# christopherkarani/Wax

Measured on NVIDIA H100. Metric: queries/sec cosine top-10 @ 10Mx384 fp32, higher is better.
Workload: dtype f32

## Files before the change

### wax_b200/csrc/waxvs_batch.cuh

```cuda
#pragma once
#include <cuda.h>
#include <cuda_bf16.h>

#include "waxvs_common.cuh"
#include "waxvs_scan.cuh"

namespace waxvs {

constexpr int kBatchM = 128;
constexpr int kBatchN = 128;
constexpr int kBatchKBlock = 32;
constexpr int kBatchKBlockBf16 = 64;
constexpr int kBatchRescore = 256;
constexpr int kBatchRescoreMax = 1024;
constexpr uint32_t kBatchABytes = kBatchM * 128u;
constexpr uint32_t kBatchBBytes = kBatchN * 128u;
constexpr uint32_t kBatchStageBytes = kBatchABytes + kBatchBBytes;
constexpr int kBatchStageSlots = 8;
constexpr uint32_t kBatchScoreStride = kBatchN + 8;
constexpr uint32_t kBatchScoreBytes = kBatchM * kBatchScoreStride * 4u;
constexpr int kBatchMaxStages = 6;
constexpr uint32_t kBatchSmemOptin = 227u * 1024u;
__host__ __device__ constexpr uint32_t batch_smem_bytes(int stages, int heap, uint32_t ares_kb = 0) {
    return ares_kb * kBatchABytes + stages * (ares_kb ? kBatchBBytes : kBatchStageBytes) + kBatchScoreBytes +
// ... 897 lines not shown
            const float scale = METRIC == kCosine ? qn : qn * __uint_as_float(*p.max_norm_bits);
            const float sk_exact = METRIC == kCosine ? (1.0f - dk) * qn : 1.0f - dk;
            const float acc_slack = static_cast<float>(p.dims) * 0x1p-23f * scale;
            const float ulp_slack = 0x1p-21f * fmaxf(1.0f, fabsf(dk)) * (METRIC == kCosine ? qn : 1.0f);
            const float eps = p.eps_rel * scale * 1.01f + acc_slack + ulp_slack + 1e-30f;
            if (excluded_any && (!(sk_exact > tau + eps) || !finite_f32(eps))) ok = 0;
            const float feps = kTf32Eps * scale * 1.01f + acc_slack + ulp_slack + 1e-30f;
            const float t = sk_exact - feps;
            tau_star = finite_f32(t) ? t - fabsf(t) * 0x1p-20f - 1e-30f : -INFINITY;
            const float feps16 = kBf16Eps * scale * 1.01f + acc_slack + ulp_slack + 1e-30f;
            const float t16 = sk_exact - feps16;
            tau_star16 = finite_f32(t16) ? t16 - fabsf(t16) * 0x1p-20f - 1e-30f : -INFINITY;
        } else if (excluded_any) {
            ok = 0;
        }
        if (METRIC != kL2 && (!(s_a2 >= 0x1p-126f) || !finite_f32(s_a2))) {
            ok = 0;
            tau_star = tau_star16 = -INFINITY;
        }
        p.ok[q] = ok;
        if (p.tau_star) { p.tau_star[q] = tau_star; p.tau_star[p.tau_stride + q] = tau_star16; }
    }
    ScanParams sp{};
    sp.out = p.out + static_cast<size_t>(q) * p.k;
    sp.frame_ids = p.frame_ids; sp.id_base = p.id_base; sp.row_offset = p.row_offset; sp.row_keys = p.row_keys;
    for (uint32_t i = threadIdx.x; i < p.k; i += blockDim.x)
        write_candidate(sp, static_cast<int>(i), i < p.rescore ? ek[i] : WAXVS_KEY_NONE);
}

struct RescoreParams {
    const float *corpus, *query;
    uint32_t dims, k, n_nominees;
    const uint64_t *nominees;
    uint32_t *aux;
    const uint32_t *max_norm_bits;
    float rho_max;
    uint64_t *block_keys;
    uint32_t *ticket;
    uint32_t *work_counter;
    wax_vs_candidate *out;
    uint32_t *ok;
    const uint64_t *frame_ids, *row_keys;
    uint64_t id_base, row_offset;
    uint32_t tail_smem_bytes;
};

template <int METRIC>
__global__ void __launch_bounds__(512, 1) shadow_rescore_kernel(const RescoreParams p) {
    static_assert(METRIC == kCosine || METRIC == kDot, "the shadow route covers cosine and dot");
    extern __shared__ __align__(16) unsigned char rsm[];
    __shared__ float s_a2, s_sqrt_a2;
    const int warp = threadIdx.x >> 5, lane = threadIdx.x & 31, warps = blockDim.x >> 5;
    const int k = static_cast<int>(p.k);
    if (warp == 0) {
        float s0 = 0.f, s1 = 0.f, s2 = 0.f, s3 = 0.f;
        for (uint32_t base = 4u * lane; base < p.dims; base += 128u) {
            const float4 x = __ldg(reinterpret_cast<const float4 *>(p.query + base));
            s0 = __fmaf_rn(x.x, x.x, s0); s1 = __fmaf_rn(x.y, x.y, s1);
            s2 = __fmaf_rn(x.z, x.z, s2); s3 = __fmaf_rn(x.w, x.w, s3);
        }
        const float a2 = warp_butterfly_sum(__fadd_rn(__fadd_rn(s0, s1), __fadd_rn(s2, s3)));
        if (lane == 0) { s_a2 = a2; s_sqrt_a2 = __fsqrt_rn(a2); }
    }
    __shared__ ScanParams sp;
    for (uint32_t i = threadIdx.x; i < sizeof(ScanParams) / 4u; i += blockDim.x) reinterpret_cast<uint32_t *>(&sp)[i] = 0u;
    __syncthreads();
    if (threadIdx.x == 0) {
        sp.k = p.k; sp.block_keys = p.block_keys; sp.ticket = p.ticket; sp.out = p.out;
        sp.frame_ids = p.frame_ids; sp.id_base = p.id_base; sp.row_offset = p.row_offset; sp.row_keys = p.row_keys;
        sp.tail_smem_bytes = p.tail_smem_bytes; sp.work_counter = p.work_counter;
    }
    __syncthreads();

    WarpTopK<1> tk;
    tk.init();
    const uint32_t stride = gridDim.x * warps * 4u;
    for (uint32_t i0 = (blockIdx.x * warps + warp) * 4u; i0 < p.n_nominees; i0 += stride) {
        uint64_t nk[4];
        const float *vp[4];
        float d[4];
#pragma unroll
        for (uint32_t r = 0; r < 4; ++r) {
            nk[r] = i0 + r < p.n_nominees ? p.nominees[i0 + r] : WAXVS_KEY_NONE;
            vp[r] = p.corpus + static_cast<size_t>(nk[r] == WAXVS_KEY_NONE ? 0u : static_cast<uint32_t>(nk[r])) * p.dims;
        }
        exact_row_distance_x4<METRIC>(p.query, vp, p.dims, s_a2, s_sqrt_a2, lane, d);
#pragma unroll
        for (uint32_t r = 0; r < 4; ++r) {
            if (nk[r] == WAXVS_KEY_NONE || !finite_f32(d[r])) continue;
            const uint64_t x = make_key(d[r], static_cast<uint32_t>(nk[r]));
            if (x < tk.thresh) tk.insert(x, lane, k);
        }
    }

    if (!finish_topk_select<1>(sp, tk, rsm)) return;
    __syncthreads();
    if (threadIdx.x != 0) return;
    const wax_vs_candidate kth = p.out[p.k - 1];
    const uint32_t cut = p.aux[0];
    const bool excluded_any = cut != WAXVS_UKEY_NONE;
    const float tau = excluded_any ? -from_orderable_u32(cut) : -INFINITY;
    const float rho_q = __uint_as_float(p.aux[1]);
    uint32_t ok = 1;
    if (kth.valid) {
        const float dk = kth.distance, qn = s_sqrt_a2;
        const float m = METRIC == kCosine ? 1.0f : __uint_as_float(*p.max_norm_bits);
        const float scale = qn * m;
        const float sk_exact = METRIC == kCosine ? (1.0f - dk) * qn : 1.0f - dk;
        const float coding = qn * p.rho_max + rho_q * ((METRIC == kCosine ? 1.0001f : m) + p.rho_max);
        const float acc_slack = static_cast<float>(p.dims) * 0x1p-23f * scale;
        const float ulp_slack = 0x1p-21f * fmaxf(1.0f, fabsf(dk)) * (METRIC == kCosine ? qn : 1.0f);
        const float eps = coding * 1.01f + acc_slack + ulp_slack + 1e-30f;
        if (excluded_any && (!(sk_exact > tau + eps) || !finite_f32(eps))) ok = 0;
    } else if (excluded_any) {
        ok = 0;
    }
    if (!(s_a2 >= 0x1p-126f) || !finite_f32(s_a2)) ok = 0;
    *p.ok = ok;
    p.aux[0] = WAXVS_UKEY_NONE;
    p.aux[2] = cut;
}

template <int METRIC>
__global__ void __launch_bounds__(256) filter_rescore_kernel(const float *corpus, const float *queries, uint32_t dims,
                                                             const uint32_t *cand_count, const uint32_t *cand_rows,
                                                             uint32_t cand_cap, uint64_t *keys) {
    const uint32_t q = blockIdx.y;
    const int lane = threadIdx.x & 31;
    const uint32_t n = min(cand_count[q], cand_cap);
    const uint32_t warps = (gridDim.x * blockDim.x) >> 5;
    uint32_t i = (blockIdx.x * blockDim.x + threadIdx.x) >> 5;
    if (i >= n) return;
    const float *qv = queries + static_cast<size_t>(q) * dims;
    float a2 = 0.0f, sqrt_a2 = 0.0f;
    if (METRIC == kCosine) {
        float s0 = 0.f, s1 = 0.f, s2 = 0.f, s3 = 0.f;
        for (uint32_t base = 4u * lane; base < dims; base += 128u) {
            const float x = __ldg(qv + base); s0 = __fmaf_rn(x, x, s0);
            if (base + 1 < dims) { const float y = __ldg(qv + base + 1); s1 = __fmaf_rn(y, y, s1); }
            if (base + 2 < dims) { const float z = __ldg(qv + base + 2); s2 = __fmaf_rn(z, z, s2); }
            if (base + 3 < dims) { const float w = __ldg(qv + base + 3); s3 = __fmaf_rn(w, w, s3); }
        }
        a2 = warp_butterfly_sum(__fadd_rn(__fadd_rn(s0, s1), __fadd_rn(s2, s3)));
        sqrt_a2 = __fsqrt_rn(a2);
    }
    for (uint32_t i0 = i; i0 < n; i0 += 4u * warps) {
        uint32_t rr[4];
        const float *vp[4];
        float d[4];
#pragma unroll
        for (uint32_t r = 0; r < 4; ++r) {
            const uint32_t j = i0 + r * warps;
            rr[r] = cand_rows[static_cast<size_t>(q) * cand_cap + (j < n ? j : i0)];
// ... 43 lines not shown
```

### wax_b200/csrc/waxvs_engine.cu

```cuda
#include <cuda_runtime.h>

#include <algorithm>
#include <atomic>
#include <cstdarg>
#include <cstdio>
#include <cstring>
#include <limits>
#include <map>
#include <mutex>
#include <new>
#include <shared_mutex>
#include <string>
#include <unordered_map>
#include <chrono>
#include <random>
#include <thread>
#include <unistd.h>
#include <cmath>
#include <vector>

#include "../../include/wax_vs_cuda.h"
#include "waxvs_common.cuh"
#include "waxvs_scan.cuh"
#include "waxvs_select.cuh"
// ... 780 lines not shown
}

constexpr uint32_t kShadowNominees = 128;
constexpr uint32_t kShadowRescore = 256;
constexpr uint32_t kShadowSkipQueries = 16;
static bool shadow_route_applies(const wax_vs_engine *e) {
    return e->tune.shadow_scan && (e->similarity == WAX_VS_COSINE || e->similarity == WAX_VS_DOT) && !e->debug_trace &&
           e->tune.batch_bf16 != 0 && e->dims % kBatchKBlockBf16 == 0 &&
           e->n_rows * e->dims * sizeof(float) >= e->tune.route[kRouteBf16].min_bytes;
}
static int32_t select_route_form(wax_vs_engine *e, cudaStream_t stream, bool demoted, bool *use, RouteForm *form,
                                 TmaConfig *cfg) {
    *use = false;
    for (const RouteForm f : {kRouteU4, kRouteInt8, kRouteBf16}) {
        if ((f == kRouteU4 && demoted) || e->n_rows * e->dims * sizeof(float) < e->tune.route[f].min_bytes ||
            !pick_route_config(e, f, cfg))
            continue;
        if (const int32_t rc = ensure_route_shadow(e, f, stream)) return rc;
        if (e->shadows[f].valid && e->shadows[f].eps_rel <= kRouteSpec[f].max_eps_rel) {
            *use = true;
            *form = f;
            return WAX_VS_OK;
        }
    }
    return WAX_VS_OK;
}

static int32_t enqueue_shadow_nominations(wax_vs_engine *e, SearchCtx *c, const ScanParams &p, const TmaConfig &cfg,
                                          cudaStream_t stream, uint64_t *launches, uint32_t *shape, RouteForm f) {
    const RouteFormSpec &fs = kRouteSpec[f];
    const wax_vs_engine::Shadow &sh = e->shadows[f];
    int32_t rc;
    if (fs.grid_rescore && !c->d_u4_aux) {
        if ((rc = c->d_u4_aux.ensure(3, "4-bit route state"))) return rc;
        CUDA_TRY(cudaMemsetAsync(c->d_u4_aux, 0xFF, 3 * sizeof(uint32_t), stream));
    }
    const size_t cta_keys = static_cast<size_t>(std::max(e->tune.grid, e->sm_count)) * kU4CtaNominees;
    if ((rc = c->d_heaps.ensure(std::max(static_cast<size_t>(kShadowNominees) * kNomineeStride, fs.grid_rescore ? cta_keys : 0), "nominee keys")) ||
        (rc = c->d_ok.ensure(1, "proof flags")) || (!p.query && (rc = c->d_queries.ensure(e->dims, "query buffer"))))
        return rc;

    ScanParams sp = p;
    sp.corpus = reinterpret_cast<const float *>(sh.codes.p);
    sp.row_scale = fs.scaled ? sh.scale.p : nullptr;
    sp.u4_aux = fs.grid_rescore ? c->d_u4_aux.p : nullptr;
    sp.k = kShadowNominees;
    sp.out = nullptr; sp.host_out = nullptr; sp.host_flag = nullptr;
    sp.nominees = c->d_heaps;
    sp.query_store = p.query ? nullptr : c->d_queries.p;
    sp.tail_select = e->tune.tail_select ? 1u : 0u;
    sp.tail_smem_bytes = static_cast<uint32_t>(static_cast<size_t>(cfg.warps) * cfg.stages * cfg.R * e->dims * fs.tail_bytes);
    const int grid = tma_grid(e, c, cfg, sp);
    CUDA_TRY(fs.launch(e, &sp, grid, cfg, e->similarity, stream));

    if (fs.grid_rescore) {
        RescoreParams rp{};
        rp.corpus = e->d_corpus; rp.query = p.query ? p.query : c->d_queries.p;
        rp.dims = e->dims; rp.k = p.k; rp.n_nominees = static_cast<uint32_t>(grid) * kU4CtaNominees;
        rp.nominees = c->d_heaps; rp.aux = c->d_u4_aux; rp.max_norm_bits = e->d_max_norm; rp.rho_max = sh.rho_max;
        rp.block_keys = c->d_block_keys; rp.ticket = c->d_ticket; rp.work_counter = sp.work_counter; rp.out = p.out; rp.ok = c->d_ok;
        rp.frame_ids = p.frame_ids; rp.id_base = p.id_base; rp.row_offset = p.row_offset; rp.row_keys = p.row_keys;
        rp.tail_smem_bytes = static_cast<uint32_t>(grid) * p.k * sizeof(uint64_t);
        if (rp.tail_smem_bytes > 48u * 1024u) rp.tail_smem_bytes = 0;
        const auto kernel = e->similarity == WAX_VS_COSINE ? shadow_rescore_kernel<kCosine> : shadow_rescore_kernel<kDot>;
        kernel<<<grid, 512, rp.tail_smem_bytes, stream>>>(rp);
        CUDA_TRY(cudaGetLastError());
    } else {
        FinishParams fp{};
        fp.corpus = e->d_corpus; fp.queries = p.query ? p.query : c->d_queries.p;
        fp.n_rows = p.n_rows; fp.dims = e->dims; fp.n_queries = 1; fp.groups = 1; fp.slices = 1;
        fp.kprime = kShadowNominees; fp.k = p.k; fp.metric = e->similarity;
        fp.heaps = c->d_heaps; fp.max_norm_bits = e->d_max_norm;
        fp.out = p.out; fp.ok = c->d_ok;
        fp.frame_ids = p.frame_ids; fp.id_base = p.id_base; fp.row_offset = p.row_offset; fp.row_keys = p.row_keys;
        fp.pow2_all = 512; fp.rescore = kShadowRescore; fp.eps_rel = sh.eps_rel;
        const size_t fsmem = static_cast<size_t>(fp.pow2_all + fp.rescore) * sizeof(uint64_t);
        const auto kernel = e->similarity == WAX_VS_COSINE ? batch_finish_kernel<kCosine> : batch_finish_kernel<kDot>;
        CUDA_TRY(grant_smem(e, kernel, fsmem));
        kernel<<<1, 512, fsmem, stream>>>(fp);
        CUDA_TRY(cudaGetLastError());
    }
    *launches += 2;
    if (shape) {
        const uint32_t s[7] = {static_cast<uint32_t>(cfg.C), static_cast<uint32_t>(cfg.R), static_cast<uint32_t>(cfg.warps),
                               static_cast<uint32_t>(cfg.stages), static_cast<uint32_t>(grid), sp.chunk_steps, sp.tail_select};
        std::copy(s, s + 7, shape);
    }
    return WAX_VS_OK;
}

static int32_t enqueue_shadow_route(wax_vs_engine *e, SearchCtx *c, ScanParams &p, cudaStream_t stream, uint64_t *launches) {
    if (!shadow_route_applies(e)) return WAX_VS_OK;
    int32_t rc;
    if (!c->h_proof_count) {
        if ((rc = c->d_proof_count.ensure(2, "proof counts")) || (rc = c->h_proof_count.ensure(2, "proof count mirror"))) return rc;
        CUDA_TRY(cudaMemsetAsync(c->d_proof_count, 0, 2 * sizeof(uint32_t), stream));
        c->h_proof_count[0] = c->h_proof_count[1] = 0;
        c->seen_failed = 0;
    }
    bool demoted;
    {
        std::lock_guard<std::mutex> pg(e->pool_mu);
        const uint32_t failed = *static_cast<volatile uint32_t *>(c->h_proof_count + 1);
        if (failed != c->seen_failed) {
            c->seen_failed = failed;
            if (c->last_u4) {
                if (e->u4_probing) e->u4_demote_window = std::min(e->u4_demote_window * 2, 1u << 20);
                e->u4_demoted = e->u4_demote_window;
            } else {
                e->shadow_scan_skip = kShadowSkipQueries;
            }
        } else if (c->last_u4 && e->u4_probing) {
            e->u4_demote_window = 16;
        }
        if (c->last_u4) e->u4_probing = false;
        c->last_u4 = false;
        if (e->shadow_scan_skip > 0) { --e->shadow_scan_skip; return WAX_VS_OK; }
        demoted = e->u4_demoted > 0;
        if (demoted && --e->u4_demoted == 0) e->u4_probing = true;
    }
    bool use = false;
    RouteForm form = kRouteBf16;
    TmaConfig cfg{};
    if ((rc = select_route_form(e, stream, demoted, &use, &form, &cfg)) || !use) return rc;
    if ((rc = enqueue_shadow_nominations(e, c, p, cfg, stream, launches, nullptr, form))) return rc;
    c->last_u4 = form == kRouteU4;
    {
        std::lock_guard<std::mutex> pg(e->pool_mu);
        ++e->single_route_queries[form];
    }
// ... 4630 lines not shown
    else if (!strcmp(name, "batch_bf16_queries")) *out = e->batch_bf16_queries;
    else if (!strcmp(name, "batch_retry_queries")) *out = e->batch_retry_queries;
    else if (!strcmp(name, "batch_filter_bf16_queries")) *out = e->batch_filter_bf16_queries;
    else if (!strcmp(name, "shadow_bytes")) *out = bf.valid ? bf.rows * e->dims * sizeof(__nv_bfloat16) : 0;
    else if (!strcmp(name, "shadow_capacity_bytes")) *out = bf.codes.cap * sizeof(uint32_t);
    else if (!strcmp(name, "shadow_unavailable")) *out = bf.unavailable ? 1 : 0;
    else if (!strcmp(name, "batch_tf32_queries")) *out = e->batch_tf32_queries;
    else if (!strcmp(name, "filter_bitset_passes")) *out = e->filter_bitset_passes;
    else if (!strcmp(name, "group_index_builds")) *out = e->group_index_builds;
    else if (!strcmp(name, "where_group_units")) *out = e->where_group_units;
    else if (!strcmp(name, "where_group_rows_walked")) *out = e->where_group_rows_walked;
    else if (!strcmp(name, "attribute_uploads")) *out = e->attribute_uploads;
    else if (!strcmp(name, "location_uploads")) *out = e->location_uploads;
    else if (!strcmp(name, "term_index_builds")) *out = e->term_index_builds;
    else if (!strcmp(name, "term_index_bytes"))
        *out = e->tindex.keys.cap * sizeof(uint64_t) + e->tindex.start.cap * sizeof(uint64_t) + e->tindex.postings.cap * sizeof(uint32_t);
    else if (!strcmp(name, "grouped_batch_covered_queries")) *out = e->grouped_batch_covered_queries;
    else if (!strcmp(name, "grouped_batch_expanded_groups")) *out = e->grouped_batch_expanded_groups;
    else if (!strcmp(name, "grouped_batch_fallback_queries")) *out = e->grouped_batch_fallback_queries;
    else if (!strcmp(name, "grouped_batch_expansion_passes")) *out = e->grouped_batch_expansion_passes;
    else if (!strcmp(name, "shard_grouped_expanded_groups")) *out = e->shard_grouped_expanded_groups;
    else if (!strcmp(name, "ingest_h2d_bytes")) *out = e->ingest_h2d_bytes;
    else if (!strcmp(name, "ingest_d2h_bytes")) *out = e->ingest_d2h_bytes;
    else if (!strcmp(name, "norms_rows")) *out = e->norms_rows;
    else if (!strcmp(name, "shadow_rows")) *out = bf.rows;
    else if (!strcmp(name, "int8_shadow_bytes")) *out = i8.valid ? i8.rows * (e->dims + sizeof(float)) : 0;
    else if (!strcmp(name, "int8_shadow_rows")) *out = i8.rows;
    else if (!strcmp(name, "u4_shadow_bytes")) *out = u4.valid ? u4.rows * (e->dims / 2 + sizeof(float)) : 0;
    else if (!strcmp(name, "u4_shadow_rows")) *out = u4.rows;
    else if (!strcmp(name, "single_u4_queries")) *out = e->single_route_queries[kRouteU4];
    else if (!strcmp(name, "single_int8_queries")) *out = e->single_route_queries[kRouteInt8];
    else if (!strcmp(name, "batch_heap_bump")) *out = e->heap_bump;
    else if (!strcmp(name, "batch_last_heap")) *out = e->last_heap;
    else if (!strcmp(name, "single_shadow_queries") || !strcmp(name, "single_shadow_fallbacks")) {
        const int slot = !strcmp(name, "single_shadow_queries") ? 0 : 1;
        uint64_t n = 0;
        auto add = [&](const SearchCtx *c) { if (c->h_proof_count) n += *static_cast<volatile uint32_t *>(c->h_proof_count + slot); };
        for (const SearchCtx *c : e->pool) add(c);
        for (const auto &kv : e->stream_ctx) add(kv.second);
        *out = n;
    }
    else if (!strcmp(name, "pool_allocs")) *out = e->pool_allocs;
    else if (!strcmp(name, "pool_reuses")) *out = e->pool_reuses;
    else return fail(WAX_VS_ERR_ARGUMENT, "unknown counter '%s'", name);
    return WAX_VS_OK;
}

int32_t wax_vs_debug_time_search_batch(wax_vs_engine *e, uint32_t n_queries, int64_t top_k, uint64_t seed,
                                       uint32_t warmup, uint32_t iters, float *out_ms_total,
                                       uint64_t *out_launches, uint32_t *out_unproven) {
    WAX_VS_MULTI_REFUSE(e, "wax_vs_debug_time_search_batch");
    if (!e || !out_ms_total) return fail(WAX_VS_ERR_NULL, "NULL argument");
    if (n_queries == 0) n_queries = 1;
    std::shared_lock<std::shared_mutex> r(e->rw);
    DeviceGuard g(e->device);
    const uint32_t k_eff = static_cast<uint32_t>(std::min<uint64_t>(clamp_topk(top_k), std::max<uint64_t>(e->n_rows, 1)));
    if (!batch_tensor_eligible(e, n_queries, k_eff))
        return fail(WAX_VS_ERR_UNSUPPORTED, "batch of %u queries, k=%u, dims=%u is not eligible for the tensor path", n_queries, k_eff, e->dims);
    CtxLease lease(e);
    int32_t rc = lease.acquire();
    if (rc) return rc;
    SearchCtx *c = lease.c;
    const size_t qfloats = static_cast<size_t>(n_queries) * e->dims;
    if ((rc = c->d_queries.ensure(qfloats, "query buffer"))) return rc;
    if ((rc = c->d_out.ensure(static_cast<size_t>(n_queries) * k_eff, "result buffer"))) return rc;
    if ((rc = c->d_ok.ensure(static_cast<size_t>(n_queries), "proof flags"))) return rc;
    if ((rc = c->h_ok.ensure(static_cast<size_t>(n_queries), "proof flag staging"))) return rc;
    synth_fill_kernel<<<(n_queries + 255) / 256, 256, 0, c->stream>>>(c->d_queries, n_queries, e->dims, seed, 0, 1);
// ... 86 lines not shown
        e->tune.batch_bf16 == 0 || e->dims % kBatchKBlockBf16 != 0 ||
        (form == kRouteBf16 && e->shadows[kRouteBf16].unavailable) || !pick_route_config(e, form, &cfg))
        return fail(WAX_VS_ERR_UNSUPPORTED, "no %s-shadow route for k=%u, dims=%u in this shape", fs.name, k_eff, e->dims);
    DeviceGuard g(e->device);
    if (!g.ok) return g.error();
    CtxLease lease(e);
    int32_t rc = lease.acquire();
    if (rc) return rc;
    SearchCtx *c = lease.c;
    if ((rc = ensure_route_shadow(e, form, c->stream, true))) return rc;
    if (!e->shadows[form].valid) return fail(WAX_VS_ERR_UNSUPPORTED, "the %s shadow does not fit in device memory", fs.name);
    if ((rc = c->d_out.ensure(k_eff, "result buffer"))) return rc;
    const uint32_t *d_mask = nullptr;
    if (allow_bits) {
        const size_t words = static_cast<size_t>((e->n_rows + 31) / 32);
        if ((rc = c->d_mask.ensure(words, "row filter"))) return rc;
        CUDA_TRY(cudaMemcpyAsync(c->d_mask, allow_bits, words * sizeof(uint32_t), cudaMemcpyHostToDevice, c->stream));
        d_mask = c->d_mask;
    }
    ScanParams p = scan_params(e, c, nullptr, k_eff, 0, c->d_out, nullptr, d_mask);
    if ((rc = place_host_query(e, c, p, query, true, c->stream))) return rc;
    uint64_t launches = 0;
    if ((rc = enqueue_shadow_nominations(e, c, p, cfg, c->stream, &launches, out_shape, form))) {
        cudaStreamSynchronize(c->stream);
        return rc;
    }
    CUDA_TRY(cudaStreamSynchronize(c->stream));
    if (fs.grid_rescore) {
        const uint64_t n_keys = static_cast<uint64_t>(out_shape[4]) * kU4CtaNominees;
        if (keys_cap < n_keys)
            return fail(WAX_VS_ERR_BUFFER, "the nominees need %llu entries (%llu given)", static_cast<unsigned long long>(n_keys),
                        static_cast<unsigned long long>(keys_cap));
        CUDA_TRY(cudaMemcpy(out_keys, c->d_heaps, n_keys * sizeof(uint64_t), cudaMemcpyDeviceToHost));
        uint32_t aux[3];
        CUDA_TRY(cudaMemcpy(aux, c->d_u4_aux, sizeof aux, cudaMemcpyDeviceToHost));
        out_bound[0] = e->shadows[form].rho_max;
        memcpy(out_bound + 1, &aux[1], sizeof(float));
        if (aux[2] == 0xFFFFFFFFu) out_bound[2] = -INFINITY;
        else { const uint32_t u = aux[2] ^ ((aux[2] & 0x80000000u) ? 0x80000000u : 0xFFFFFFFFu); float f; memcpy(&f, &u, 4); out_bound[2] = -f; }
    } else {
        CUDA_TRY(cudaMemcpy2D(out_keys, sizeof(uint64_t), c->d_heaps, kNomineeStride * sizeof(uint64_t), sizeof(uint64_t),
                              kShadowNominees, cudaMemcpyDeviceToHost));
    }
    CUDA_TRY(cudaMemcpy(out_ok, c->d_ok, sizeof(uint32_t), cudaMemcpyDeviceToHost));
    CUDA_TRY(cudaMemcpy(out_result, c->d_out, k_eff * sizeof(wax_vs_candidate), cudaMemcpyDeviceToHost));
    for (uint32_t i = 0; i < k_eff; ++i)
        if (out_result[i].valid) out_result[i].frame_id = frame_id_of(e, out_result[i].row);
    return WAX_VS_OK;
}

int32_t wax_vs_debug_shadow_nominations(wax_vs_engine *e, const float *query, int64_t top_k, const uint32_t *allow_bits,
                                        uint64_t *out_keys, uint32_t *out_ok, wax_vs_candidate *out_result,
                                        uint32_t *out_shape) {
    WAX_VS_MULTI_REFUSE(e, "wax_vs_debug_shadow_nominations");
    return debug_route_nominations(e, query, top_k, allow_bits, out_keys, out_ok, out_result, out_shape, kRouteBf16);
}

int32_t wax_vs_debug_int8_nominations(wax_vs_engine *e, const float *query, int64_t top_k, const uint32_t *allow_bits,
                                      uint64_t *out_keys, uint32_t *out_ok, wax_vs_candidate *out_result,
                                      uint32_t *out_shape) {
    WAX_VS_MULTI_REFUSE(e, "wax_vs_debug_int8_nominations");
    return debug_route_nominations(e, query, top_k, allow_bits, out_keys, out_ok, out_result, out_shape, kRouteInt8);
}

int32_t wax_vs_debug_u4_nominations(wax_vs_engine *e, const float *query, int64_t top_k, const uint32_t *allow_bits,
                                    uint64_t *out_keys, uint64_t keys_cap, uint32_t *out_ok, wax_vs_candidate *out_result,
                                    uint32_t *out_shape, float *out_bound) {
    WAX_VS_MULTI_REFUSE(e, "wax_vs_debug_u4_nominations");
    return debug_route_nominations(e, query, top_k, allow_bits, out_keys, out_ok, out_result, out_shape, kRouteU4,
                                   keys_cap, out_bound);
}

// ... 118 lines not shown
```

### wax_b200/csrc/waxvs_scan.cuh

```cuda
#pragma once
#include "waxvs_common.cuh"
#include "waxvs_shard.cuh"
#include "../../include/wax_vs_cuda.h"

namespace waxvs {

constexpr int kInlineQueryFloats = 512;

struct ScanParams {
    const float *corpus;
    const float *query;
    uint32_t n_rows;
    uint32_t dims;
    uint32_t k;
    uint32_t stages;
    uint64_t *block_keys;
    uint32_t *ticket;
    wax_vs_candidate *out;
    uint32_t *dist_keys;
    const uint64_t *frame_ids;
    uint64_t id_base;
    uint64_t row_offset;
    const uint64_t *row_keys;
    uint32_t use_l2_hint;
    uint32_t chunk_steps;
    uint32_t *work_counter;
    const uint32_t *mask;
    wax_vs_candidate *host_out;
    unsigned long long *host_flag;
    unsigned long long host_seq;
    alignas(16) float query_inline[kInlineQueryFloats];
    uint32_t tail_select;
    uint32_t tail_smem_bytes;
    unsigned long long *trace;
    ShardParams shard;
    uint64_t *nominees;
    float *query_store;
    const uint32_t *proof_ok;
    uint32_t *proof_count;
    uint32_t *proof_count_host;
    const float *row_scale;
    uint32_t *u4_aux;
};

constexpr uint32_t kU4CtaNominees = 256;

constexpr int kNomineeStride = 128;

__device__ __forceinline__ bool row_allowed(const ScanParams &p, uint32_t row) {
    return p.mask == nullptr || ((__ldg(p.mask + (row >> 5)) >> (row & 31u)) & 1u) != 0u;
}

__device__ __forceinline__ void write_candidate(const ScanParams &p, int slot, uint64_t key) {
    wax_vs_candidate c;
    if (key == WAXVS_KEY_NONE) {
        c.distance = 0.0f; c.valid = 0; c.row = 0; c.frame_id = 0;
    } else {
        const uint32_t row = static_cast<uint32_t>(key);
        c.distance = from_orderable_u32(static_cast<uint32_t>(key >> 32));
        c.valid = 1;
        c.row = p.row_offset + (p.row_keys ? p.row_keys[row] : row);
        c.frame_id = p.frame_ids ? p.frame_ids[row] : p.id_base + row;
    }
    p.out[slot] = c;
    if (p.host_out) p.host_out[slot] = c;
}

template <bool SHADOW>
__device__ __forceinline__ void write_slot(const ScanParams &p, int slot, uint64_t key) {
    if constexpr (SHADOW) p.nominees[static_cast<size_t>(slot == static_cast<int>(p.k) - 1 ? 0 : slot + 1) * kNomineeStride] = key;
    else write_candidate(p, slot, key);
}

__device__ __forceinline__ float4 bf16x4_to_float4(uint2 u) {
    return make_float4(__uint_as_float(u.x << 16), __uint_as_float(u.x & 0xFFFF0000u),
// ... 187 lines not shown
    auto grid_keys = [&](auto f) {
        if (staged) { for (uint32_t i = tid; i < total; i += nthr) f(sk[i]); }
        else { for (uint32_t i = tid; i < total; i += nthr) f(ld_cg_u64(p.block_keys + i)); }
    };
    const uint64_t xb = block_select_kth(grid_keys, k, &ss);
    if (tid == 0) ss.n_sel = 0;
    __syncthreads();
    grid_keys([&](uint64_t key) { if (key != WAXVS_KEY_NONE && key <= xb) ss.sel[atomicAdd(&ss.n_sel, 1u)] = key; });
    __syncthreads();
    const uint32_t n_sel = ss.n_sel;
    for (uint32_t i = tid; i < k; i += nthr) {
        if (i < n_sel) {
            const uint64_t key = ss.sel[i];
            uint32_t rank = 0;
            for (uint32_t j = 0; j < n_sel; ++j) rank += ss.sel[j] < key ? 1u : 0u;
            write_slot<SHADOW>(p, static_cast<int>(rank), key);
        } else {
            write_slot<SHADOW>(p, static_cast<int>(i), WAXVS_KEY_NONE);
        }
    }
    if (p.host_flag && !p.shard.world) __threadfence_system();
    __syncthreads();
    if (tid == 0) {
        *p.ticket = 0u;
        if (p.work_counter) *p.work_counter = 0u;
        if (p.host_flag && !p.shard.world) st_release_sys_u64(p.host_flag, p.host_seq);
        if (p.trace) p.trace[4] = global_timer_ns();
    }
    if (p.shard.world) shard_exchange_cta(p.shard, p.out, p.k, reinterpret_cast<uint32_t *>(scratch));
    return true;
}

template <int E>
__device__ __forceinline__ void finish_u4_nominees(const ScanParams &p, WarpTopK<E> &tk) {
    __shared__ SelectScratch ss;
    __shared__ uint32_t s_cut;
    const uint32_t tid = threadIdx.x, nthr = blockDim.x;
    if (tid == 0) s_cut = WAXVS_UKEY_NONE;
    auto own_keys = [&](auto f) {
#pragma unroll
        for (int j = 0; j < E; ++j) f(tk.key[j]);
    };
    const uint64_t xa = nthr * E >= kU4CtaNominees ? block_select_kth(own_keys, kU4CtaNominees, &ss) : WAXVS_KEY_NONE;
    if (tid == 0) ss.n_sel = 0;
    __syncthreads();
    uint64_t *mine = p.nominees + static_cast<size_t>(blockIdx.x) * kU4CtaNominees;
#pragma unroll
    for (int j = 0; j < E; ++j)
        if (tk.key[j] != WAXVS_KEY_NONE && tk.key[j] <= xa) mine[atomicAdd(&ss.n_sel, 1u)] = tk.key[j];
    if ((tid & 31u) == 0 && tk.thresh != WAXVS_KEY_NONE) atomicMin(&s_cut, static_cast<uint32_t>(tk.thresh >> 32));
    __syncthreads();
    for (uint32_t i = ss.n_sel + tid; i < kU4CtaNominees; i += nthr) mine[i] = WAXVS_KEY_NONE;
    if (tid == 0) {
        uint32_t cut = s_cut;
        if (xa != WAXVS_KEY_NONE) cut = min(cut, static_cast<uint32_t>(xa >> 32));
        if (cut != WAXVS_UKEY_NONE) atomicMin(p.u4_aux, cut);
    }
}

template <int C, int R, int METRIC, int E, bool EMIT, bool SHADOW = false, bool INT8 = false, bool U4 = false>
__global__ void __launch_bounds__(512, 1) scan_tma_kernel(const __grid_constant__ ScanParams p) {
    static_assert(!SHADOW || (C > 0 && METRIC != kL2 && !EMIT), "the shadow form covers the unrolled cosine / dot shapes");
    static_assert(!INT8 || (SHADOW && R >= 4), "the int8 form is a shadow form with 16-byte scale copies");
    static_assert(!U4 || (SHADOW && !INT8 && R >= 4 && E == 4), "the 4-bit form is a shadow form with 16-byte scale copies");
    constexpr bool SCALED = INT8 || U4;
    if constexpr (!SHADOW && !EMIT && E == 1 && METRIC != kL2) {
        if (p.proof_ok) {
            const bool proven = *p.proof_ok != 0u;
            if (blockIdx.x == 0) {
                if (threadIdx.x == 0) {
                    const uint32_t n = ++p.proof_count[proven ? 0 : 1];
                    *static_cast<volatile uint32_t *>(p.proof_count_host + (proven ? 0 : 1)) = n;
                }
                if (proven && p.host_flag) {
                    for (uint32_t i = threadIdx.x; i < p.k; i += blockDim.x) p.host_out[i] = p.out[i];
                    __threadfence_system();
                    __syncthreads();
                    if (threadIdx.x == 0) st_release_sys_u64(p.host_flag, p.host_seq);
                }
            }
            if (proven) return;
        }
    }
    const int D4 = C > 0 ? 32 * C : static_cast<int>(p.dims / 4u);
    const int CN = C > 0 ? C : (D4 + 31) / 32;
    const uint32_t ROW_BYTES = C > 0 ? (U4 ? 64u : INT8 ? 128u : SHADOW ? 256u : 512u) * C : p.dims * 4u;
    const uint32_t STAGE_BYTES = ROW_BYTES * R + (SCALED ? R * 4u : 0u);
    constexpr int LANES_PER_ROW = 32 / R;

    extern __shared__ __align__(128) unsigned char smem[];
// ... 256 lines not shown
        else d = finish_l2(sum0[0]);
        if (SHADOW && !finite_f32(d)) d = -INFINITY;
        const bool leader = U4 ? (hl % (16 / H)) == 0 : (lane % LANES_PER_ROW) == 0;
        const bool ok = (my_row < p.n_rows) && (SHADOW || finite_f32(d));

        if (EMIT) {
            if (leader && my_row < p.n_rows)
                p.dist_keys[my_row] = (ok && row_allowed(p, my_row)) ? orderable_u32(d) : WAXVS_UKEY_NONE;
        } else {
            const uint64_t key = ok ? make_key(d, my_row) : WAXVS_KEY_NONE;
            const bool cand = leader && key < tk.thresh && row_allowed(p, my_row);
            uint32_t m = __ballot_sync(WAXVS_FULL_MASK, cand);
            if (E == 1) {
                while (m) {
                    const int src = __ffs(m) - 1;
                    m &= m - 1;
                    const uint64_t x = shfl_u64(key, src);
                    if (x < tk.thresh) tk.insert(x, lane, k);
                }
            } else if (m) {
                if (tk.npend + __popc(m) > 32) tk.flush(lane, k);
                while (m) {
                    const int src = __ffs(m) - 1;
                    m &= m - 1;
                    tk.park(shfl_u64(key, src), lane);
                }
            }
        }
    }

    if (p.trace && lane == 0) atomicMax(p.trace + 1, global_timer_ns());
    if (!EMIT) {
        if (E > 1) tk.flush(lane, k);
        if constexpr (U4) finish_u4_nominees<E>(p, tk);
        else if (p.tail_select) finish_topk_select<E, SHADOW>(p, tk, smem);
        else finish_topk<E, SHADOW>(p, tk, lists, warp, lane, warps);
    }
}

template <int METRIC, int E, bool EMIT>
__global__ void __launch_bounds__(256, 4) scan_ldg_kernel(const __grid_constant__ ScanParams p) {
    __shared__ uint64_t lists[8 * 32 * E];
    const int warp = threadIdx.x >> 5, lane = threadIdx.x & 31, warps = blockDim.x >> 5;
    const uint32_t dims = p.dims;
    const bool vec4 = (dims % 4u) == 0u;
    const uint32_t d4 = dims / 4u;

    float a2 = 0.0f, sqrt_a2 = 0.0f;
    if (METRIC == kCosine) {
        float s0 = 0.f, s1 = 0.f, s2 = 0.f, s3 = 0.f;
        for (uint32_t base = 4u * lane; base < dims; base += 128u) {
            const float x = __ldg(p.query + base);
            const float y = (base + 1 < dims) ? __ldg(p.query + base + 1) : 0.0f;
            const float z = (base + 2 < dims) ? __ldg(p.query + base + 2) : 0.0f;
            const float w = (base + 3 < dims) ? __ldg(p.query + base + 3) : 0.0f;
            s0 = __fmaf_rn(x, x, s0);
            if (base + 1 < dims) s1 = __fmaf_rn(y, y, s1);
            if (base + 2 < dims) s2 = __fmaf_rn(z, z, s2);
            if (base + 3 < dims) s3 = __fmaf_rn(w, w, s3);
        }
        a2 = warp_butterfly_sum(__fadd_rn(__fadd_rn(s0, s1), __fadd_rn(s2, s3)));
        sqrt_a2 = __fsqrt_rn(a2);
    }

    WarpTopK<E> tk;
    tk.init();
    const int k = static_cast<int>(p.k);
    const uint32_t total_warps = gridDim.x * warps;
// ... 57 lines not shown
```

### wax_b200/engine.py

```python
from __future__ import annotations

import ctypes as C
import dataclasses
import enum
import threading
from typing import Iterable, List, NamedTuple, Optional, Sequence, Tuple

import numpy as np

from . import _lib as L


class WaxError(Exception):
    pass


class EncodingError(WaxError):
    pass


class CapacityExceeded(WaxError):
    pass


# ... 938 lines not shown
            mask = np.zeros(((n + 31) // 32) * 32, bool)
            mask[np.asarray(allow_rows, np.int64)] = True
            bits = (mask.reshape(-1, 32).astype(np.uint64) << np.arange(32, dtype=np.uint64)).sum(1).astype(np.uint32)
        u32 = lambda a: a.ctypes.data_as(C.POINTER(C.c_uint32))
        heaps = np.empty(0, np.uint64)
        for _ in range(2):
            rc = L.lib().wax_vs_debug_batch_nominations(
                self._h, q.ctypes.data_as(C.POINTER(C.c_float)), nq, int(top_k), None if bits is None else u32(bits),
                scores.ctypes.data_as(C.POINTER(C.c_float)), u32(ok),
                heaps.ctypes.data_as(C.POINTER(C.c_uint64)) if heaps.size else None, heaps.size, u32(shape))
            if rc != L.ERR_BUFFER or heaps.size:
                break
            heaps = np.empty(int(shape[5]) * int(shape[6]) * int(shape[4]) * 128, np.uint64)
        _check(rc)
        names = ("bf16", "ares", "pair", "stages", "kprime", "slices", "groups")
        out = {name: int(v) for name, v in zip(names, shape)}
        out.update(scores=scores, ok=ok, heaps=heaps.reshape(out["slices"] * out["groups"], out["kprime"], 128))
        return out

    def shadow_nominations(self, vector, top_k: int, allow_rows=None):
        return self._route_nominations(L.lib().wax_vs_debug_shadow_nominations, vector, top_k, allow_rows)

    def int8_nominations(self, vector, top_k: int, allow_rows=None):
        return self._route_nominations(L.lib().wax_vs_debug_int8_nominations, vector, top_k, allow_rows)

    def u4_nominations(self, vector, top_k: int, allow_rows=None):
        return self._route_nominations(L.lib().wax_vs_debug_u4_nominations, vector, top_k, allow_rows, u4=True)

    def _route_nominations(self, fn, vector, top_k: int, allow_rows, u4: bool = False):
        q = np.ascontiguousarray(vector, dtype=np.float32).reshape(self.dimensions)
        n = self.count
        k = max(1, min(int(top_k), n))
        keys = np.empty(256 * 1024 if u4 else 128, np.uint64)
        bound = np.zeros(3, np.float32)
        ok = C.c_uint32(0)
        result = (L.Candidate * k)()
        shape = np.zeros(7, np.uint32)
        bits = None
        if allow_rows is not None:
            mask = np.zeros(((n + 31) // 32) * 32, bool)
            mask[np.asarray(allow_rows, np.int64)] = True
            bits = (mask.reshape(-1, 32).astype(np.uint64) << np.arange(32, dtype=np.uint64)).sum(1).astype(np.uint32)
        u32 = lambda a: a.ctypes.data_as(C.POINTER(C.c_uint32))
        if u4:
            _check(fn(
                self._h, q.ctypes.data_as(C.POINTER(C.c_float)), int(top_k), None if bits is None else u32(bits),
                keys.ctypes.data_as(C.POINTER(C.c_uint64)), keys.size, C.byref(ok), result, u32(shape),
                bound.ctypes.data_as(C.POINTER(C.c_float))))
            keys = keys[:int(shape[4]) * 256]
        else:
            _check(fn(
                self._h, q.ctypes.data_as(C.POINTER(C.c_float)), int(top_k), None if bits is None else u32(bits),
                keys.ctypes.data_as(C.POINTER(C.c_uint64)), C.byref(ok), result, u32(shape)))
        one = np.float32(1.0)
        score = (lambda d: float(one - np.float32(d))) if self.metric is VectorMetric.cosine else (lambda d: float(-np.float32(d)))
        names = ("C", "R", "warps", "stages", "grid", "chunk_steps", "tail_select")
        out = {name: int(v) for name, v in zip(names, shape)}
        out.update(keys=keys, ok=ok.value, result=[(int(c.frame_id), score(c.distance)) for c in result if c.valid])
        if u4:
            out.update(rho_max=float(bound[0]), rho_q=float(bound[1]), tau_excl=float(bound[2]))
        return out

    def read_shadow(self, first: int, n: int) -> np.ndarray:
        out = np.empty((n, self.dimensions), np.uint16)
        _check(L.lib().wax_vs_debug_read_shadow(self._h, first, n, out.ctypes.data_as(C.POINTER(C.c_uint16))))
        return out

    def read_int8_shadow(self, first: int, n: int):
        codes = np.empty((n, self.dimensions), np.uint8)
        scales = np.empty(n, np.float32)
        rho = C.c_float(0.0)
        _check(L.lib().wax_vs_debug_read_int8_shadow(self._h, first, n, codes.ctypes.data_as(C.POINTER(C.c_uint8)),
                                                     scales.ctypes.data_as(C.POINTER(C.c_float)), C.byref(rho)))
        return codes, scales, float(rho.value)

    def read_u4_shadow(self, first: int, n: int):
        packed = np.empty((n, self.dimensions // 2), np.uint8)
        half = np.empty(n, np.float32)
        rho = C.c_float(0.0)
        _check(L.lib().wax_vs_debug_read_u4_shadow(self._h, first, n, packed.ctypes.data_as(C.POINTER(C.c_uint8)),
                                                   half.ctypes.data_as(C.POINTER(C.c_float)), C.byref(rho)))
        w = packed.reshape(n, -1, 4)
        codes = np.concatenate([w & 15, w >> 4], axis=2).reshape(n, self.dimensions)
        return codes, half, float(rho.value)

    def stream_read_gbs(self, iters: int = 5) -> float:
        ms, nbytes = C.c_float(0), C.c_uint64(0)
        _check(L.lib().wax_vs_debug_stream_read(self._h, iters, C.byref(ms), C.byref(nbytes)))
        return nbytes.value / (ms.value * 1e6) if ms.value > 0 else 0.0

    def set_option(self, key: str, value: int) -> None:
        _check(L.lib().wax_vs_debug_set_option(self._h, key.encode(), int(value)))

# ... 13 lines not shown
```

Baseline: 1499.

## Skip provably non-competitive u4 nominees using per-CTA exact best rows

Each scan CTA now computes the exact fp32 distance of its best 4-bit nominee and publishes it. The rescore kernel ranks those exact keys to get the k-th best, derives a safe skip threshold from the u4 error margin, and skips fp32 rescoring of nominees whose approximate score falls below it. Skipped nominees are folded into the exclusion bound of the proof check. The aim is to cut the fp32 corpus reads during rescoring, at the cost of one extra exact row per CTA, ballot/compaction overhead, and extra counters.

```diff
diff --git a/wax_b200/csrc/waxvs_batch.cuh b/wax_b200/csrc/waxvs_batch.cuh
--- a/wax_b200/csrc/waxvs_batch.cuh
+++ b/wax_b200/csrc/waxvs_batch.cuh
@@ -953,6 +953,8 @@
     const float *corpus, *query;
     uint32_t dims, k, n_nominees;
     const uint64_t *nominees;
+    const uint64_t *best;
+    uint32_t n_best;
     uint32_t *aux;
     const uint32_t *max_norm_bits;
     float rho_max;
@@ -961,18 +963,39 @@
     uint32_t *work_counter;
     wax_vs_candidate *out;
     uint32_t *ok;
+    uint32_t *counts, *counts_host;
     const uint64_t *frame_ids, *row_keys;
     uint64_t id_base, row_offset;
     uint32_t tail_smem_bytes;
 };
+
+constexpr uint32_t kRescoreMaxBest = 512;
+
+template <int METRIC>
+__device__ __forceinline__ float u4_proof_margin(const RescoreParams &p, float dk, float qn, float rho_q, float *sk) {
+    const float m = METRIC == kCosine ? 1.0f : __uint_as_float(*p.max_norm_bits);
+    const float scale = qn * m;
+    *sk = METRIC == kCosine ? (1.0f - dk) * qn : 1.0f - dk;
+    const float coding = qn * p.rho_max + rho_q * ((METRIC == kCosine ? 1.0001f : m) + p.rho_max);
+    const float acc_slack = static_cast<float>(p.dims) * 0x1p-23f * scale;
+    const float ulp_slack = 0x1p-21f * fmaxf(1.0f, fabsf(dk)) * (METRIC == kCosine ? qn : 1.0f);
+    return coding * 1.01f + acc_slack + ulp_slack + 1e-30f;
+}
 
 template <int METRIC>
 __global__ void __launch_bounds__(512, 1) shadow_rescore_kernel(const RescoreParams p) {
     static_assert(METRIC == kCosine || METRIC == kDot, "the shadow route covers cosine and dot");
     extern __shared__ __align__(16) unsigned char rsm[];
     __shared__ float s_a2, s_sqrt_a2;
+    __shared__ uint64_t s_best[kRescoreMaxBest];
+    __shared__ unsigned long long s_lkey;
+    __shared__ uint32_t s_skip_word, s_skipped, s_rescored;
+    __shared__ float s_sl, s_skip_below;
+    __shared__ uint64_t s_pack[16][32];
     const int warp = threadIdx.x >> 5, lane = threadIdx.x & 31, warps = blockDim.x >> 5;
     const int k = static_cast<int>(p.k);
+    const uint32_t n_best = p.n_best <= kRescoreMaxBest ? p.n_best : 0u;
+    for (uint32_t i = threadIdx.x; i < n_best; i += blockDim.x) s_best[i] = p.best[i];
     if (warp == 0) {
         float s0 = 0.f, s1 = 0.f, s2 = 0.f, s3 = 0.f;
         for (uint32_t base = 4u * lane; base < p.dims; base += 128u) {
@@ -990,56 +1013,101 @@
         sp.k = p.k; sp.block_keys = p.block_keys; sp.ticket = p.ticket; sp.out = p.out;
         sp.frame_ids = p.frame_ids; sp.id_base = p.id_base; sp.row_offset = p.row_offset; sp.row_keys = p.row_keys;
         sp.tail_smem_bytes = p.tail_smem_bytes; sp.work_counter = p.work_counter;
+        s_lkey = WAXVS_KEY_NONE; s_skip_word = WAXVS_UKEY_NONE; s_skipped = 0; s_rescored = 0;
+    }
+    __syncthreads();
+    for (uint32_t i = threadIdx.x; i < n_best; i += blockDim.x) {
+        const uint64_t x = s_best[i];
+        uint32_t rank = 0;
+        for (uint32_t j = 0; j < n_best; ++j) rank += s_best[j] < x ? 1u : 0u;
+        if (x != WAXVS_KEY_NONE && rank == p.k - 1) s_lkey = x;
+    }
+    __syncthreads();
+    if (threadIdx.x == 0) {
+        float s_l = -INFINITY, t = -INFINITY;
+        if (s_lkey != WAXVS_KEY_NONE && s_a2 >= 0x1p-126f && finite_f32(s_a2)) {
+            const float margin = u4_proof_margin<METRIC>(p, from_orderable_u32(static_cast<uint32_t>(s_lkey >> 32)),
+                                                         s_sqrt_a2, __uint_as_float(p.aux[1]), &s_l);
+            t = s_l - margin - (fabsf(s_l) + margin) * 0x1p-20f;
+        }
+        s_sl = s_l;
+        s_skip_below = finite_f32(t) ? t : -INFINITY;
     }
     __syncthreads();
 
     WarpTopK<1> tk;
     tk.init();
-    const uint32_t stride = gridDim.x * warps * 4u;
-    for (uint32_t i0 = (blockIdx.x * warps + warp) * 4u; i0 < p.n_nominees; i0 += stride) {
-        uint64_t nk[4];
-        const float *vp[4];
-        float d[4];
-#pragma unroll
-        for (uint32_t r = 0; r < 4; ++r) {
-            nk[r] = i0 + r < p.n_nominees ? p.nominees[i0 + r] : WAXVS_KEY_NONE;
-            vp[r] = p.corpus + static_cast<size_t>(nk[r] == WAXVS_KEY_NONE ? 0u : static_cast<uint32_t>(nk[r])) * p.dims;
-        }
-        exact_row_distance_x4<METRIC>(p.query, vp, p.dims, s_a2, s_sqrt_a2, lane, d);
-#pragma unroll
-        for (uint32_t r = 0; r < 4; ++r) {
-            if (nk[r] == WAXVS_KEY_NONE || !finite_f32(d[r])) continue;
-            const uint64_t x = make_key(d[r], static_cast<uint32_t>(nk[r]));
-            if (x < tk.thresh) tk.insert(x, lane, k);
-        }
+    const uint32_t gw = blockIdx.x * warps + warp, total_warps = gridDim.x * warps;
+    for (uint32_t j0 = 0; (static_cast<uint64_t>(gw) + static_cast<uint64_t>(j0 / 4u) * total_warps) * 4u < p.n_nominees;
+         j0 += 32u) {
+        const uint32_t j = j0 + lane;
+        const uint64_t idx = (static_cast<uint64_t>(gw) + static_cast<uint64_t>(j / 4u) * total_warps) * 4u + (j & 3u);
+        const uint64_t key = idx < p.n_nominees ? p.nominees[idx] : WAXVS_KEY_NONE;
+        const bool skip = key != WAXVS_KEY_NONE && -from_orderable_u32(static_cast<uint32_t>(key >> 32)) < s_skip_below;
+        if (skip) atomicMin(&s_skip_word, static_cast<uint32_t>(key >> 32));
+        const bool keep = key != WAXVS_KEY_NONE && !skip;
+        const uint32_t m = __ballot_sync(WAXVS_FULL_MASK, keep), n_keep = __popc(m);
+        const uint32_t n_skip = __popc(__ballot_sync(WAXVS_FULL_MASK, skip));
+        if (lane == 0) { atomicAdd(&s_skipped, n_skip); atomicAdd(&s_rescored, n_keep); }
+        if (keep) s_pack[warp][__popc(m & ((1u << lane) - 1u))] = key;
+        __syncwarp();
+        for (uint32_t g = 0; g < n_keep; g += 4u) {
+            uint64_t nk[4];
+            const float *vp[4];
+            float d[4];
+#pragma unroll
+            for (uint32_t r = 0; r < 4; ++r) {
+                nk[r] = g + r < n_keep ? s_pack[warp][g + r] : WAXVS_KEY_NONE;
+                vp[r] = p.corpus + static_cast<size_t>(nk[r] == WAXVS_KEY_NONE ? 0u : static_cast<uint32_t>(nk[r])) * p.dims;
+            }
+            exact_row_distance_x4<METRIC>(p.query, vp, p.dims, s_a2, s_sqrt_a2, lane, d);
+#pragma unroll
+            for (uint32_t r = 0; r < 4; ++r) {
+                if (nk[r] == WAXVS_KEY_NONE || !finite_f32(d[r])) continue;
+                const uint64_t x = make_key(d[r], static_cast<uint32_t>(nk[r]));
+                if (x < tk.thresh) tk.insert(x, lane, k);
+            }
+        }
+        __syncwarp();
+    }
+    __syncthreads();
+    if (threadIdx.x == 0) {
+        if (s_skip_word != WAXVS_UKEY_NONE) atomicMin(p.aux + 3, s_skip_word);
+        atomicAdd(p.aux + 4, s_skipped);
+        atomicAdd(p.aux + 5, s_rescored);
     }
 
     if (!finish_topk_select<1>(sp, tk, rsm)) return;
     __syncthreads();
     if (threadIdx.x != 0) return;
     const wax_vs_candidate kth = p.out[p.k - 1];
-    const uint32_t cut = p.aux[0];
-    const bool excluded_any = cut != WAXVS_UKEY_NONE;
-    const float tau = excluded_any ? -from_orderable_u32(cut) : -INFINITY;
-    const float rho_q = __uint_as_float(p.aux[1]);
+    const uint32_t cut = p.aux[0], left_out = min(cut, __ldcg(p.aux + 3));
+    const bool excluded_any = left_out != WAXVS_UKEY_NONE;
+    const float tau = excluded_any ? -from_orderable_u32(left_out) : -INFINITY;
     uint32_t ok = 1;
     if (kth.valid) {
-        const float dk = kth.distance, qn = s_sqrt_a2;
-        const float m = METRIC == kCosine ? 1.0f : __uint_as_float(*p.max_norm_bits);
-        const float scale = qn * m;
-        const float sk_exact = METRIC == kCosine ? (1.0f - dk) * qn : 1.0f - dk;
-        const float coding = qn * p.rho_max + rho_q * ((METRIC == kCosine ? 1.0001f : m) + p.rho_max);
-        const float acc_slack = static_cast<float>(p.dims) * 0x1p-23f * scale;
-        const float ulp_slack = 0x1p-21f * fmaxf(1.0f, fabsf(dk)) * (METRIC == kCosine ? qn : 1.0f);
-        const float eps = coding * 1.01f + acc_slack + ulp_slack + 1e-30f;
+        float sk_exact;
+        const float eps = u4_proof_margin<METRIC>(p, kth.distance, s_sqrt_a2, __uint_as_float(p.aux[1]), &sk_exact);
         if (excluded_any && (!(sk_exact > tau + eps) || !finite_f32(eps))) ok = 0;
     } else if (excluded_any) {
         ok = 0;
     }
     if (!(s_a2 >= 0x1p-126f) || !finite_f32(s_a2)) ok = 0;
     *p.ok = ok;
+    const uint32_t n_skipped = __ldcg(p.aux + 4), n_rescored = __ldcg(p.aux + 5);
     p.aux[0] = WAXVS_UKEY_NONE;
+    p.aux[3] = WAXVS_UKEY_NONE;
+    p.aux[4] = 0u;
+    p.aux[5] = 0u;
     p.aux[2] = cut;
+    p.aux[6] = __float_as_uint(s_sl);
+    p.aux[7] = __float_as_uint(s_skip_below);
+    p.aux[8] = n_skipped;
+    if (p.counts) {
+        const uint32_t a = p.counts[0] += n_skipped, b = p.counts[1] += n_rescored;
+        static_cast<volatile uint32_t *>(p.counts_host)[0] = a;
+        static_cast<volatile uint32_t *>(p.counts_host)[1] = b;
+    }
 }
 
 template <int METRIC>
diff --git a/wax_b200/csrc/waxvs_engine.cu b/wax_b200/csrc/waxvs_engine.cu
--- a/wax_b200/csrc/waxvs_engine.cu
+++ b/wax_b200/csrc/waxvs_engine.cu
@@ -836,11 +836,12 @@
     const wax_vs_engine::Shadow &sh = e->shadows[f];
     int32_t rc;
     if (fs.grid_rescore && !c->d_u4_aux) {
-        if ((rc = c->d_u4_aux.ensure(3, "4-bit route state"))) return rc;
-        CUDA_TRY(cudaMemsetAsync(c->d_u4_aux, 0xFF, 3 * sizeof(uint32_t), stream));
-    }
-    const size_t cta_keys = static_cast<size_t>(std::max(e->tune.grid, e->sm_count)) * kU4CtaNominees;
-    if ((rc = c->d_heaps.ensure(std::max(static_cast<size_t>(kShadowNominees) * kNomineeStride, fs.grid_rescore ? cta_keys : 0), "nominee keys")) ||
+        if ((rc = c->d_u4_aux.ensure(9, "4-bit route state"))) return rc;
+        CUDA_TRY(cudaMemsetAsync(c->d_u4_aux, 0xFF, 4 * sizeof(uint32_t), stream));
+        CUDA_TRY(cudaMemsetAsync(c->d_u4_aux + 4, 0, 5 * sizeof(uint32_t), stream));
+    }
+    const size_t max_grid = static_cast<size_t>(std::max(e->tune.grid, e->sm_count)), cta_keys = max_grid * kU4CtaNominees;
+    if ((rc = c->d_heaps.ensure(std::max(static_cast<size_t>(kShadowNominees) * kNomineeStride, fs.grid_rescore ? cta_keys + max_grid : 0), "nominee keys")) ||
         (rc = c->d_ok.ensure(1, "proof flags")) || (!p.query && (rc = c->d_queries.ensure(e->dims, "query buffer"))))
         return rc;
 
@@ -848,6 +849,9 @@
     sp.corpus = reinterpret_cast<const float *>(sh.codes.p);
     sp.row_scale = fs.scaled ? sh.scale.p : nullptr;
     sp.u4_aux = fs.grid_rescore ? c->d_u4_aux.p : nullptr;
+    sp.u4_best = fs.grid_rescore ? c->d_heaps + cta_keys : nullptr;
+    sp.u4_fp32 = e->d_corpus;
+    sp.u4_cosine = e->similarity == WAX_VS_COSINE ? 1u : 0u;
     sp.k = kShadowNominees;
     sp.out = nullptr; sp.host_out = nullptr; sp.host_flag = nullptr;
     sp.nominees = c->d_heaps;
@@ -861,9 +865,10 @@
         RescoreParams rp{};
         rp.corpus = e->d_corpus; rp.query = p.query ? p.query : c->d_queries.p;
         rp.dims = e->dims; rp.k = p.k; rp.n_nominees = static_cast<uint32_t>(grid) * kU4CtaNominees;
-        rp.nominees = c->d_heaps; rp.aux = c->d_u4_aux; rp.max_norm_bits = e->d_max_norm; rp.rho_max = sh.rho_max;
+        rp.nominees = c->d_heaps; rp.best = sp.u4_best; rp.n_best = static_cast<uint32_t>(grid); rp.aux = c->d_u4_aux; rp.max_norm_bits = e->d_max_norm; rp.rho_max = sh.rho_max;
         rp.block_keys = c->d_block_keys; rp.ticket = c->d_ticket; rp.work_counter = sp.work_counter; rp.out = p.out; rp.ok = c->d_ok;
         rp.frame_ids = p.frame_ids; rp.id_base = p.id_base; rp.row_offset = p.row_offset; rp.row_keys = p.row_keys;
+        if (c->h_proof_count) { rp.counts = c->d_proof_count + 2; rp.counts_host = c->h_proof_count + 2; }
         rp.tail_smem_bytes = static_cast<uint32_t>(grid) * p.k * sizeof(uint64_t);
         if (rp.tail_smem_bytes > 48u * 1024u) rp.tail_smem_bytes = 0;
         const auto kernel = e->similarity == WAX_VS_COSINE ? shadow_rescore_kernel<kCosine> : shadow_rescore_kernel<kDot>;
@@ -897,9 +902,9 @@
     if (!shadow_route_applies(e)) return WAX_VS_OK;
     int32_t rc;
     if (!c->h_proof_count) {
-        if ((rc = c->d_proof_count.ensure(2, "proof counts")) || (rc = c->h_proof_count.ensure(2, "proof count mirror"))) return rc;
-        CUDA_TRY(cudaMemsetAsync(c->d_proof_count, 0, 2 * sizeof(uint32_t), stream));
-        c->h_proof_count[0] = c->h_proof_count[1] = 0;
+        if ((rc = c->d_proof_count.ensure(4, "proof counts")) || (rc = c->h_proof_count.ensure(4, "proof count mirror"))) return rc;
+        CUDA_TRY(cudaMemsetAsync(c->d_proof_count, 0, 4 * sizeof(uint32_t), stream));
+        for (int i = 0; i < 4; ++i) c->h_proof_count[i] = 0;
         c->seen_failed = 0;
     }
     bool demoted;
@@ -5596,8 +5601,10 @@
     else if (!strcmp(name, "single_int8_queries")) *out = e->single_route_queries[kRouteInt8];
     else if (!strcmp(name, "batch_heap_bump")) *out = e->heap_bump;
     else if (!strcmp(name, "batch_last_heap")) *out = e->last_heap;
-    else if (!strcmp(name, "single_shadow_queries") || !strcmp(name, "single_shadow_fallbacks")) {
-        const int slot = !strcmp(name, "single_shadow_queries") ? 0 : 1;
+    else if (!strcmp(name, "single_shadow_queries") || !strcmp(name, "single_shadow_fallbacks") ||
+             !strcmp(name, "u4_skipped_nominees") || !strcmp(name, "u4_rescored_nominees")) {
+        const int slot = !strcmp(name, "single_shadow_queries") ? 0 : !strcmp(name, "single_shadow_fallbacks") ? 1
+                       : !strcmp(name, "u4_skipped_nominees") ? 2 : 3;
         uint64_t n = 0;
         auto add = [&](const SearchCtx *c) { if (c->h_proof_count) n += *static_cast<volatile uint32_t *>(c->h_proof_count + slot); };
         for (const SearchCtx *c : e->pool) add(c);
@@ -5750,12 +5757,14 @@
             return fail(WAX_VS_ERR_BUFFER, "the nominees need %llu entries (%llu given)", static_cast<unsigned long long>(n_keys),
                         static_cast<unsigned long long>(keys_cap));
         CUDA_TRY(cudaMemcpy(out_keys, c->d_heaps, n_keys * sizeof(uint64_t), cudaMemcpyDeviceToHost));
-        uint32_t aux[3];
+        uint32_t aux[9];
         CUDA_TRY(cudaMemcpy(aux, c->d_u4_aux, sizeof aux, cudaMemcpyDeviceToHost));
         out_bound[0] = e->shadows[form].rho_max;
         memcpy(out_bound + 1, &aux[1], sizeof(float));
         if (aux[2] == 0xFFFFFFFFu) out_bound[2] = -INFINITY;
         else { const uint32_t u = aux[2] ^ ((aux[2] & 0x80000000u) ? 0x80000000u : 0xFFFFFFFFu); float f; memcpy(&f, &u, 4); out_bound[2] = -f; }
+        memcpy(out_bound + 3, &aux[6], 2 * sizeof(float));
+        out_bound[5] = static_cast<float>(aux[8]);
     } else {
         CUDA_TRY(cudaMemcpy2D(out_keys, sizeof(uint64_t), c->d_heaps, kNomineeStride * sizeof(uint64_t), sizeof(uint64_t),
                               kShadowNominees, cudaMemcpyDeviceToHost));
diff --git a/wax_b200/csrc/waxvs_scan.cuh b/wax_b200/csrc/waxvs_scan.cuh
--- a/wax_b200/csrc/waxvs_scan.cuh
+++ b/wax_b200/csrc/waxvs_scan.cuh
@@ -41,6 +41,9 @@
     uint32_t *proof_count_host;
     const float *row_scale;
     uint32_t *u4_aux;
+    uint64_t *u4_best;
+    const float *u4_fp32;
+    uint32_t u4_cosine;
 };
 
 constexpr uint32_t kU4CtaNominees = 256;
@@ -294,11 +297,12 @@
 }
 
 template <int E>
-__device__ __forceinline__ void finish_u4_nominees(const ScanParams &p, WarpTopK<E> &tk) {
+__device__ __forceinline__ uint64_t finish_u4_nominees(const ScanParams &p, WarpTopK<E> &tk) {
     __shared__ SelectScratch ss;
     __shared__ uint32_t s_cut;
+    __shared__ unsigned long long s_best;
     const uint32_t tid = threadIdx.x, nthr = blockDim.x;
-    if (tid == 0) s_cut = WAXVS_UKEY_NONE;
+    if (tid == 0) { s_cut = WAXVS_UKEY_NONE; s_best = WAXVS_KEY_NONE; }
     auto own_keys = [&](auto f) {
 #pragma unroll
         for (int j = 0; j < E; ++j) f(tk.key[j]);
@@ -311,6 +315,12 @@
     for (int j = 0; j < E; ++j)
         if (tk.key[j] != WAXVS_KEY_NONE && tk.key[j] <= xa) mine[atomicAdd(&ss.n_sel, 1u)] = tk.key[j];
     if ((tid & 31u) == 0 && tk.thresh != WAXVS_KEY_NONE) atomicMin(&s_cut, static_cast<uint32_t>(tk.thresh >> 32));
+    uint64_t best = tk.key[0];
+#pragma unroll
+    for (int j = 1; j < E; ++j) best = min(best, tk.key[j]);
+#pragma unroll
+    for (int o = 16; o > 0; o >>= 1) best = min(best, static_cast<uint64_t>(__shfl_xor_sync(WAXVS_FULL_MASK, best, o)));
+    if ((tid & 31u) == 0 && best != WAXVS_KEY_NONE) atomicMin(&s_best, static_cast<unsigned long long>(best));
     __syncthreads();
     for (uint32_t i = ss.n_sel + tid; i < kU4CtaNominees; i += nthr) mine[i] = WAXVS_KEY_NONE;
     if (tid == 0) {
@@ -318,6 +328,36 @@
         if (xa != WAXVS_KEY_NONE) cut = min(cut, static_cast<uint32_t>(xa >> 32));
         if (cut != WAXVS_UKEY_NONE) atomicMin(p.u4_aux, cut);
     }
+    return s_best;
+}
+
+template <int C, typename LoadQ>
+__device__ __forceinline__ void u4_best_exact(const ScanParams &p, uint64_t best, int lane, LoadQ load_q) {
+    uint64_t key = WAXVS_KEY_NONE;
+    if (best != WAXVS_KEY_NONE) {
+        const uint32_t row = static_cast<uint32_t>(best);
+        const float4 *v4 = reinterpret_cast<const float4 *>(p.u4_fp32 + static_cast<size_t>(row) * p.dims);
+        float a0 = 0.f, a1 = 0.f, a2 = 0.f, a3 = 0.f, b0 = 0.f, b1 = 0.f, b2 = 0.f, b3 = 0.f;
+        float n0 = 0.f, n1 = 0.f, n2 = 0.f, n3 = 0.f;
+#pragma unroll
+        for (int c = 0; c < C; ++c) {
+            const float4 x = __ldg(v4 + lane + 32 * c), y = load_q(lane + 32 * c);
+            a0 = __fmaf_rn(y.x, x.x, a0); a1 = __fmaf_rn(y.y, x.y, a1); a2 = __fmaf_rn(y.z, x.z, a2); a3 = __fmaf_rn(y.w, x.w, a3);
+            b0 = __fmaf_rn(x.x, x.x, b0); b1 = __fmaf_rn(x.y, x.y, b1); b2 = __fmaf_rn(x.z, x.z, b2); b3 = __fmaf_rn(x.w, x.w, b3);
+            n0 = __fmaf_rn(y.x, y.x, n0); n1 = __fmaf_rn(y.y, y.y, n1); n2 = __fmaf_rn(y.z, y.z, n2); n3 = __fmaf_rn(y.w, y.w, n3);
+        }
+        const float s0 = warp_butterfly_sum(__fadd_rn(__fadd_rn(a0, a1), __fadd_rn(a2, a3)));
+        float d;
+        if (p.u4_cosine) {
+            const float s1 = warp_butterfly_sum(__fadd_rn(__fadd_rn(b0, b1), __fadd_rn(b2, b3)));
+            const float q2 = warp_butterfly_sum(__fadd_rn(__fadd_rn(n0, n1), __fadd_rn(n2, n3)));
+            d = finish_cos(s0, q2, __fsqrt_rn(q2), s1);
+        } else {
+            d = finish_dot(s0);
+        }
+        if (finite_f32(d)) key = make_key(d, row);
+    }
+    if (lane == 0) p.u4_best[blockIdx.x] = key;
 }
 
 template <int C, int R, int METRIC, int E, bool EMIT, bool SHADOW = false, bool INT8 = false, bool U4 = false>
@@ -640,8 +680,10 @@
     if (p.trace && lane == 0) atomicMax(p.trace + 1, global_timer_ns());
     if (!EMIT) {
         if (E > 1) tk.flush(lane, k);
-        if constexpr (U4) finish_u4_nominees<E>(p, tk);
-        else if (p.tail_select) finish_topk_select<E, SHADOW>(p, tk, smem);
+        if constexpr (U4) {
+            const uint64_t best = finish_u4_nominees<E>(p, tk);
+            if (warp == 0) u4_best_exact<C>(p, best, lane, load_q);
+        } else if (p.tail_select) finish_topk_select<E, SHADOW>(p, tk, smem);
         else finish_topk<E, SHADOW>(p, tk, lists, warp, lane, warps);
     }
 }
diff --git a/wax_b200/engine.py b/wax_b200/engine.py
--- a/wax_b200/engine.py
+++ b/wax_b200/engine.py
@@ -994,7 +994,7 @@
         n = self.count
         k = max(1, min(int(top_k), n))
         keys = np.empty(256 * 1024 if u4 else 128, np.uint64)
-        bound = np.zeros(3, np.float32)
+        bound = np.zeros(6, np.float32)
         ok = C.c_uint32(0)
         result = (L.Candidate * k)()
         shape = np.zeros(7, np.uint32)
@@ -1020,7 +1020,8 @@
         out = {name: int(v) for name, v in zip(names, shape)}
         out.update(keys=keys, ok=ok.value, result=[(int(c.frame_id), score(c.distance)) for c in result if c.valid])
         if u4:
-            out.update(rho_max=float(bound[0]), rho_q=float(bound[1]), tau_excl=float(bound[2]))
+            out.update(rho_max=float(bound[0]), rho_q=float(bound[1]), tau_excl=float(bound[2]), s_l=float(bound[3]),
+                       skip_below=float(bound[4]), skipped=int(bound[5]))
         return out
 
     def read_shadow(self, first: int, n: int) -> np.ndarray:
```

Measured after the change: 1508, median of 6. Within noise of the previous version (+0.6%).
